# kvarq/kvarq

Measured on AMD Instinct MI355X. Metric: fastq_reads_per_sec_scanned, higher is better.
Workload: dtype u8

## Files before the change

### kvarq_amd/csrc/kernels_bp_pass.inc

```
#if BP_STRAIGHT
        {
            const uint32_t pass0 = 0;
#else
        for (uint32_t pass0 = 0; pass0 < nrec; pass0 += RP) {
#endif
            const uint32_t k = pass0 + gr;
            const bool have = k < nrec;
            uint32_t roff = 0; int rl = 0;
            constexpr bool late_probes = !BP_STRAIGHT && LG >= 0 && !DENSE;
            uint32_t c0, cp;
            if (have) {
                const uint32_t m = jn + 4u * k;
                const uint32_t rstart = m == 0 ? ST_PRE + (Ja & 15u) : (uint32_t)S.nl[m - 1] + 1u;
                const uint32_t n0 = S.nl[m], n1 = S.nl[m + 1], n2 = S.nl[m + 2], n3 = S.nl[m + 3];
                const uint32_t sread = n0 + 1u, plus = n1 + 1u, sscore = n2 + 1u;
        KVQ_MARK("trim" BP_SFX);
                if (gl == 0 && !late_probes) { if (dbg & 8u) { c0 = '@'; cp = '+'; } else { c0 = text[rstart]; cp = text[plus]; } }
                const int Q = (int)(n3 - sscore);
                const int per = (Q + (int)G - 1) >> lg;
                Seg sg; sg.beg = (int)mul_u24(gl, (uint32_t)per); if (sg.beg > Q) sg.beg = Q;
                int s1 = sg.beg + per; if (s1 > Q) s1 = Q;
                sg.len = 0; sg.pre = 0; sg.suf = 0; sg.best = 0; sg.bstart = sg.beg;
                {
                    auto round = [&](int c0_) -> Seg {
                        const int n = s1 - c0_ < 64 ? s1 - c0_ : 64;
                        const uint32_t bit = sscore + (uint32_t)c0_;
                        const uint32_t a = BP_LDS_GDP + ((bit >> 5) << 2), sh = bit & 31u;
                        const uint32_t d0 = lds_u32_at(a), d1 = lds_u32_at(a + 4u), d2 = lds_u32_at(a + 8u);
                        const uint64_t nmask = n < 64 ? (1ull << n) - 1ull : ~0ull;
                        const uint64_t mm = (((uint64_t)__builtin_amdgcn_alignbit(d2, d1, sh) << 32) | (uint64_t)__builtin_amdgcn_alignbit(d1, d0, sh)) & nmask;
                        Seg sub; sub.beg = c0_; sub.len = n;
                        int bs;
                        bp_runs64(mm, n, dbg, sub.pre, sub.suf, sub.best, bs);
                        sub.bstart = c0_ + bs;
                        return sub;
                    };
                    if (!__any(per > 64)) sg = round(sg.beg);
                    else {
                        for (int cc = sg.beg; cc < s1; cc += 64) {
                            const Seg sub = round(cc);
                            sg = (cc == sg.beg) ? sub : seg_merge(sg, sub);
                        }
                    }
                }
                if (G == 4u) {
#define KVQ_QUAD(v, ctl) __builtin_amdgcn_update_dpp(0, (v), (ctl), 0xf, 0xf, true)
                    {
                        Seg B;
                        B.len = KVQ_QUAD(sg.len, 0xB1); B.pre = KVQ_QUAD(sg.pre, 0xB1); B.suf = KVQ_QUAD(sg.suf, 0xB1);
                        B.best = KVQ_QUAD(sg.best, 0xB1); B.bstart = KVQ_QUAD(sg.bstart, 0xB1); B.beg = 0;
                        sg = seg_merge(sg, B);
                    }
                    {
                        Seg B;
                        B.len = KVQ_QUAD(sg.len, 0x4E); B.pre = KVQ_QUAD(sg.pre, 0x4E); B.suf = KVQ_QUAD(sg.suf, 0x4E);
                        B.best = KVQ_QUAD(sg.best, 0x4E); B.bstart = KVQ_QUAD(sg.bstart, 0x4E); B.beg = 0;
                        sg = seg_merge(sg, B);
                    }
                    rl = KVQ_QUAD(sg.best, 0x00);
                    roff = sread + (uint32_t)KVQ_QUAD(sg.bstart, 0x00);
#undef KVQ_QUAD
                } else {
                    for (uint32_t d = 1; d < G; d <<= 1) {
                        Seg B;
                        B.len = __shfl_xor(sg.len, (int)d, 64); B.pre = __shfl_xor(sg.pre, (int)d, 64); B.suf = __shfl_xor(sg.suf, (int)d, 64);
                        B.best = __shfl_xor(sg.best, (int)d, 64); B.bstart = __shfl_xor(sg.bstart, (int)d, 64); B.beg = 0;
                        if ((gl & d) == 0) sg = seg_merge(sg, B);
                    }
                    rl = __shfl(sg.best, lane & ~(int)(G - 1u), 64);
                    roff = sread + (uint32_t)__shfl(sg.bstart, lane & ~(int)(G - 1u), 64);
                }
                my_longest = my_longest > (uint32_t)(rl + 1) ? my_longest : (uint32_t)(rl + 1);
                if (gl == 0) {
                    if (rl < KVQ_RL_BINS && !recount) atomicAdd(&S.hist[rl >> 1], 1u << (16 * (rl & 1)));
                    S.rinfo[k] = roff | ((uint32_t)rl << 16);
                }
            }
        KVQ_MARK("trim end / filter" BP_SFX);
            BSTAMP(4);
            KVQ_SETPRIO(2);
            const uint32_t rpw = 64u >> lg, grw = (uint32_t)lane >> lg;
            const uint32_t wfirst = pass0 + wave * rpw;
            const uint32_t npass = wfirst < nrec ? (nrec - wfirst < rpw ? nrec - wfirst : rpw) : 0u;
            uint32_t *const q1 = S.q1 + wave * BP_QW; uint32_t *const q2 = S.q2 + wave * BP_Q2W;
            uint32_t sub = (dbg & 128u) ? npass : 0u, step = rpw;
#if BP_STRAIGHT
            if (sub < npass) {
#else
            while (sub < npass) {
#endif
                BTALLY(6, lane == 0);
                asm volatile("" : "+v"(rl), "+v"(roff));
                int minrl, me_; const __attribute__((address_space(1))) uint8_t *bmL;
                {
                    const BpArgsPtr A = bp_args(A_);
                    minrl = A->P.minreadlength; me_ = A->P.maxerrors;
                    bmL = (const __attribute__((address_space(1))) uint8_t *)A->X.bm1 + (1 << (2 * KK)) / 8;
                }
                const bool mine = have && rl >= minrl && !(dbg & 2u) && grw >= sub && grw - sub < step;
                uint32_t qn = 0;
                int e0 = 0, e1 = 0;
                if (mine) {
                    const int NPe = (rl - KK) / SS + 1;
                    const int per = (NPe + (int)G - 1) >> lg;
                    e0 = (int)mul_u24(gl, (uint32_t)per); if (e0 > NPe) e0 = NPe;
                    e1 = e0 + per; if (e1 > NPe) e1 = NPe;
                }
                auto fixed_block = [&](int pp, bool ok) -> bool {
                    const uint32_t code = cdp_code<KK>(roff + (uint32_t)(ok ? pp : 0));
                    const uint32_t bits = bmL[code >> 3];
                    return ok & (bool)((bits >> (code & 7u)) & 1u);
                };
                auto head_ok = [&](int jj) { return mine && jj <= me_ && (jj + 1) * KK <= rl; };
                auto tail_ok = [&](int jj) { const int pp = rl - (jj + 1) * KK; return mine && jj <= me_ && pp >= 0 && !((pp % KK) == 0 && pp <= me_ * KK); };
                const bool hhit = fixed_block((int)gl * KK, head_ok((int)gl));
                const bool thit = fixed_block(rl - ((int)gl + 1) * KK, tail_ok((int)gl));
                constexpr int NR = SS == 8 ? 6 : SS == 4 ? 12 : (LG == 3 || LG == 1) ? 24 : 18;
                bool first = true;
                if constexpr (!DENSE) {
                for (int ee = e0; __any(ee < e1); ee += NR, first = false) {
                    const bool act = ee < e1;
#include "kernels_bp_lookup.inc"
                    const int nv = act ? (e1 - ee < NR ? e1 - ee : NR) : 0;
                    hA &= (1u << nv) - 1u;
                    const bool hh = first && hhit, th = first && thit;
                    const uint32_t c = (uint32_t)__popc(hA) + (hh ? 1u : 0u) + (th ? 1u : 0u);
                    const uint32_t inc = kvq_wave_incl_scan(c);
                    const uint32_t tot = (uint32_t)__builtin_amdgcn_readlane((int)inc, 63);
                    if (tot) {
                        uint32_t idx = qn + inc - c;
                        while (hA) {
                            const int j = __ffs((int)hA) - 1; hA &= hA - 1u;
                            if (idx < BP_QW) q1[idx] = k | ((uint32_t)(SS * (ee + j)) << 9);
                            idx++;
                        }
                        if (hh) { if (idx < BP_QW) q1[idx] = k | ((gl * KK) << 9) | (1u << BP_Q1_KIND); idx++; }
                        if (th && idx < BP_QW) { const uint32_t pt = (uint32_t)(rl - ((int)gl + 1) * KK); q1[idx] = k | (pt << 9) | (1u << BP_Q1_KIND); }
                        qn += tot;
                    }
                }
                for (int t = (int)G; t <= me_; t += (int)G) {
                    const int jj = t + (int)gl;
#pragma unroll
                    for (int side = 0; side < 2; side++) {
                        const int pp = side ? rl - (jj + 1) * KK : jj * KK;
                        const bool hit = fixed_block(pp, side ? tail_ok(jj) : head_ok(jj));
                        const uint64_t mm = __ballot(hit);
                        if (mm) {
                            const uint32_t idx = qn + (uint32_t)__popcll(mm & kvq_lanemask_lt());
                            if (hit && idx < BP_QW) q1[idx] = k | ((uint32_t)pp << 9) | (1u << BP_Q1_KIND);
                            qn += (uint32_t)__popcll(mm);
                        }
                    }
                }
                }
        KVQ_MARK("filter end / P4a" BP_SFX);
                BSTAMP(5);
                KVQ_SETPRIO(3);

                if constexpr (!DENSE) {
                const bool over = qn > BP_QW;
                const uint32_t qn_ok = (over || (dbg & 1u)) ? 0u : qn;
#if BP_STRAIGHT
                if (over) bail = true;
                else {
#else
                if (over && step > 1u) { step >>= 1; continue; }
                if (over) {
                    if (mine && gl == 0) {
                        const BpArgsPtr A = bp_args(A_);
                        const KvqRedo Rd(A->redo);
                        const uint32_t boff = g0 - ST_PRE + roff;
                        bool put = false;
                        if (A->redo) {
                            if (rl >= KVQ_LONG_READ) {
                                const unsigned int i = atomicAdd(Rd.count + 1, 1u);
                                if (i < KVQ_LONG_CAP) { Rd.read_off[KVQ_REDO_CAP - 1u - i] = boff; Rd.read_len[KVQ_REDO_CAP - 1u - i] = rl; put = true; }
                            }
                            if (!put) {
                                const unsigned int i = atomicAdd(Rd.count, 1u);
                                if (i < A->redo_cap) { Rd.rec_start[i] = KVQ_REDO_TRIMMED; Rd.read_off[i] = boff; Rd.read_len[i] = rl; }
                                put = true;
                            }
                        }
                        if (!put) S.fallback = 1u;
                        else atomicOr(A->fail, 2u);
                    }
                }
#endif
#include "kernels_bp_p4.inc"
#if BP_STRAIGHT
                }
#endif
                } else {
                    uint32_t hA = 0, hpos = 0, tpos = 0; bool hh = false, th = false;
                    int ee = e0, xt = (int)G;
                    int ee_of_hA = e0;
                    bool done = false;
                    while (!done) {
                        bool full = false;
                        while (!full) {
                            if (!__any(hA != 0u || hh || th)) {
                                ee_of_hA = ee;
                                if (__any(ee < e1)) {
                                    const bool act = ee < e1;
                                    uint32_t hA_;
                                    {
#include "kernels_bp_lookup.inc"
                                        hA_ = hA;
                                    }
                                    const int nv = act ? (e1 - ee < NR ? e1 - ee : NR) : 0;
                                    hA = hA_ & ((1u << nv) - 1u);
                                    if (first) { hh = hhit; th = thit; hpos = gl * KK; tpos = (uint32_t)(rl - ((int)gl + 1) * KK); first = false; }
                                    ee += NR;
                                } else if (xt <= me_) {
                                    const int jj = xt + (int)gl;
                                    hpos = (uint32_t)(jj * KK); tpos = (uint32_t)(rl - (jj + 1) * KK);
                                    hh = fixed_block((int)hpos, head_ok(jj)); th = fixed_block((int)tpos, tail_ok(jj));
                                    xt += (int)G;
                                } else { done = true; break; }
                                continue;
                            }
                            const uint32_t c = (uint32_t)__popc(hA) + (hh ? 1u : 0u) + (th ? 1u : 0u);
                            const uint32_t inc = kvq_wave_incl_scan(c);
                            const uint32_t tot = (uint32_t)__builtin_amdgcn_readlane((int)inc, 63);
                            uint32_t idx = qn + inc - c;
                            while (hA && idx < BP_QW) {
                                const int j = __ffs((int)hA) - 1; hA &= hA - 1u;
                                q1[idx++] = k | ((uint32_t)(SS * (ee_of_hA + j)) << 9);
                            }
                            if (hh && idx < BP_QW) { q1[idx++] = k | (hpos << 9) | (1u << BP_Q1_KIND); hh = false; }
                            if (th && idx < BP_QW) { q1[idx++] = k | (tpos << 9) | (1u << BP_Q1_KIND); th = false; }
                            full = qn + tot >= BP_QW;
                            qn = qn + tot < BP_QW ? qn + tot : BP_QW;
                        }
                        {
                            const uint32_t qn_ok = (dbg & 1u) ? 0u : qn;
#include "kernels_bp_p4.inc"
                        }
                        qn = 0;
                    }
                }
                KVQ_SETPRIO(2);
                sub += step;
            }
            KVQ_SETPRIO(0);
            if (have && gl == 0) {
                const uint32_t m = jn + 4u * k;
                if constexpr (late_probes) {
                    if (!(dbg & 8u)) {
                        c0 = text[m == 0 ? ST_PRE + (Ja & 15u) : (uint32_t)S.nl[m - 1] + 1u];
                        cp = c0 == '@' ? (uint32_t)text[(uint32_t)S.nl[m + 1] + 1u] : (uint32_t)'+';
                    } else { c0 = '@'; cp = '+'; }
                }
                if (!bail && (c0 != '@' || cp != '+')) {
                    const BpArgsPtr A = bp_args(A_);
                    const uint32_t rstart = m == 0 ? ST_PRE + (Ja & 15u) : (uint32_t)S.nl[m - 1] + 1u, plus = (uint32_t)S.nl[m + 1] + 1u;
                    const int64_t tf = A->fpos_base + (int64_t)g0;
                    if (c0 != '@') atomicMin(A->P.err, ((unsigned long long)(tf + rstart - ST_PRE) << 16) | (0ull << 8) | c0);
                    else atomicMin(A->P.err, ((unsigned long long)(tf + plus - ST_PRE) << 16) | (1ull << 8) | cp);
                }
            }
        KVQ_MARK("P4 end" BP_SFX);
            BSTAMP(6);
        }
```

### kvarq_amd/csrc/kernels_seeded.hip

```cpp
#include "kvq_host.h"

#include <algorithm>
#include <string.h>

#ifdef KVQ_NO_PRIO
#define KVQ_SETPRIO(n) ((void)0)
#else
#define KVQ_SETPRIO(n) __builtin_amdgcn_s_setprio(n)
#endif
#define KVQ_K_MAX 8
#define ST_TILE 36640u
#define ST_TILE_MIN 30960u
#define ST_OV 4160u
#define ST_PRE 80u
#define ST_THREADS 512
#define ST_WAVES (ST_THREADS / 64)
#define ST_ROUNDS ((ST_TILE + ST_OV) / 16u / ST_THREADS + 1)
#define ST_NLCAP 2048
#define ST_RCAP 512
#define ST_QCAP 896
#define ST_Q2CAP 2048
#define ST_QW (ST_QCAP / ST_WAVES)
#define ST_Q2W (ST_Q2CAP / ST_WAVES)
#define ST_BLK 80u
#define ST_BUF (ST_PRE + ST_TILE + ST_OV)
#define ST_HIST_TILES 100u

#define TR_NONE 0xFFu
#define TR_FLAG_FALLBACK 0x2000000u
#define TR_FLAG_SKIPPED 0x4000000u
#define TR_FLAG_PARTIAL 0x8000000u
#define KVQ_SKIP_CAP 1024u

struct SeedEntry { uint64_t en, ctx; };
struct SeedTables {
    const uint32_t *bm1;
    const uint32_t *start;
    const SeedEntry *ent;
    const uint32_t *tab2;
    int32_t stride;
    int32_t pitch;
};

struct SeedIndex {
    int stride = 2;
    int k = 8;
    int pitch = 8;
    bool dense = false;
    DevBuf d_bm1, d_start, d_ent, d_tab2;
    SeedTables dev;
};

__host__ __device__ static inline uint32_t code2_of(uint8_t c) { return (c >> 1) & 3u; }

static uint32_t host_code(const uint8_t *p, int K)
{
    uint32_t c = 0;
    for (int i = 0; i < K; i++) c |= code2_of(p[i]) << (2 * i);
    return c;
}

int kvq_seed_k(const kvq_config &cfg)
{
    const int e = cfg.maxerrors;
    if (e < 0 || e > 6) return 0;
    if (cfg.Amin <= 13) return 0;
    int K = std::min(cfg.minoverlap, cfg.minreadlength) / (e + 1);
    if (K > KVQ_K_MAX) K = KVQ_K_MAX;
    if (const char *kv = getenv("KVQ_K")) { const int w = atoi(kv); if (w >= 5 && w < K) K = w; }
    return K >= 5 ? K : 0;
}

SeedIndex *kvq_seed_index_build(kvq_table *t)
{
    const kvq_config &cfg = t->cfg;
    t->seed_k = 0;
    const int e = cfg.maxerrors;
    const int K = kvq_seed_k(cfg);
    if (!K) return nullptr;
    auto pitch_of = [&](int stride) { return (K + stride - 1) / stride * stride; };
    auto span_of = [&](int stride) { return pitch_of(stride) * e + K + stride - 1; };
    int minlen = 1 << 30;
    for (int s = 0; s < t->nseq; s++) {
        const int len = t->h_off[s + 1] - t->h_off[s];
        bool ok = len >= span_of(2) && len <= 4095 && t->h_off[s] < (1 << 20) && s < (1 << 20);
        for (int i = 0; ok && i < len; i++) {
            const uint8_t c = t->h_tab[t->h_off[s] + i];
            ok = (c == 'A' || c == 'C' || c == 'G' || c == 'T');
        }
        if (ok) { t->seeded.push_back(s); t->is_seeded[s] = 1; minlen = std::min(minlen, len); }
    }
    if (t->seeded.empty()) return nullptr;
    t->seed_k = K;
    int stride = minlen >= span_of(8) ? 8 : minlen >= span_of(4) ? 4 : 2;
    if (const char *sv = getenv("KVQ_STRIDE")) { const int w = atoi(sv); if ((w == 2 || w == 4 || w == 8) && w <= stride) stride = w; }

    const int pitch = pitch_of(stride);
    struct Ent { uint32_t key; SeedEntry e; };
    std::vector<Ent> v;
    for (int s : t->seeded) {
        const uint8_t *q = &t->h_tab[t->h_off[s]];
        const int len = t->h_off[s + 1] - t->h_off[s];
        const uint64_t hi = ((uint64_t)(uint32_t)t->h_off[s] << 32) | ((uint64_t)(uint32_t)len << 52) | ((uint64_t)(uint32_t)s << 12);
        auto entry = [&](int pos, uint32_t all) -> Ent {
            uint64_t ctx = 0;
            for (int i = 0; i < 32; i++) { const int sp = pos - 16 + i; if (sp >= 0 && sp < len) ctx |= (uint64_t)code2_of(q[sp]) << (2 * i); }
            return Ent{ host_code(q + pos, K) + (all << (2 * K)), SeedEntry{ hi | (uint64_t)pos, ctx } };
        };
        for (int j = 0; j <= e; j++)
            for (int sft = 0; sft < stride; sft++) v.push_back(entry(j * pitch + sft, 0u));
        for (int p = 0; p + K <= len; p++) v.push_back(entry(p, 1u));
    }
    if (v.size() >= (1u << 22)) {
        t->seeded.clear(); std::fill(t->is_seeded.begin(), t->is_seeded.end(), 0); t->seed_k = 0;
        return nullptr;
    }
    SeedIndex *ix = new SeedIndex();
    ix->stride = stride; ix->k = K; ix->pitch = pitch;
    const uint32_t NC = 1u << (2 * K);
    std::vector<uint8_t> bm1(2 * NC / 8 < 64 ? 64 : 2 * NC / 8, 0);
    std::stable_sort(v.begin(), v.end(), [](const Ent &a, const Ent &b) { return a.key < b.key; });
    std::vector<uint32_t> start(2 * (size_t)NC + 2, 0); std::vector<SeedEntry> ent(v.size() + 1, SeedEntry{ 0, 0 });
    for (size_t i = 0; i < v.size(); i++) {
        bm1[v[i].key >> 3] |= (uint8_t)(1u << (v[i].key & 7));
        start[v[i].key + 1]++; ent[i] = v[i].e;
    }
    {
        size_t occ_anc = 0, occ_all = 0;
        for (uint32_t c = 0; c < NC; c++) { occ_anc += start[c + 1] != 0; occ_all += start[NC + c + 1] != 0; }
        const double expect = (double)occ_anc / NC * (150.0 / stride) + (double)occ_all / NC * 2 * (e + 1);
        ix->dense = expect > 5.0;
    }
    for (uint32_t c = 0; c < 2 * NC; c++) start[c + 1] += start[c];
    start[2 * (size_t)NC + 1] = start[2 * (size_t)NC];
    if (ix->d_start.ensure(start.size() * 4) != KVQ_OK || ix->d_ent.ensure(ent.size() * sizeof(SeedEntry)) != KVQ_OK ||
        hipMemcpy(ix->d_start.p, start.data(), start.size() * 4, hipMemcpyHostToDevice) != hipSuccess ||
        hipMemcpy(ix->d_ent.p, ent.data(), ent.size() * sizeof(SeedEntry), hipMemcpyHostToDevice) != hipSuccess ||
        ix->d_bm1.ensure(bm1.size()) != KVQ_OK || hipMemcpy(ix->d_bm1.p, bm1.data(), bm1.size(), hipMemcpyHostToDevice) != hipSuccess) {
        if (!kvq_error_code()) kvq_set_error(KVQ_ERR_DEVICE, "uploading the seed index failed");
        kvq_seed_index_destroy(ix);
        return nullptr;
    }
    ix->dev.bm1 = ix->d_bm1.as<uint32_t>();
    {
        const size_t nb = t->h_tab.size();
        std::vector<uint32_t> t2(nb / 16 + 3, 0);
        for (size_t i = 0; i < nb; i++) t2[i >> 4] |= code2_of(t->h_tab[i]) << (2 * (i & 15));
        if (ix->d_tab2.ensure(t2.size() * 4) != KVQ_OK || hipMemcpy(ix->d_tab2.p, t2.data(), t2.size() * 4, hipMemcpyHostToDevice) != hipSuccess) {
            if (!kvq_error_code()) kvq_set_error(KVQ_ERR_DEVICE, "uploading the seed index failed");
            kvq_seed_index_destroy(ix);
            return nullptr;
        }
        ix->dev.tab2 = ix->d_tab2.as<uint32_t>();
    }
    ix->dev.start = ix->d_start.as<uint32_t>(); ix->dev.ent = ix->d_ent.as<SeedEntry>();
    ix->dev.stride = stride; ix->dev.pitch = pitch;
    return ix;
}

void kvq_seed_index_destroy(SeedIndex *ix)
{
    if (!ix) return;
    DevBuf *b[] = { &ix->d_tab2, &ix->d_bm1, &ix->d_start, &ix->d_ent };
    for (DevBuf *x : b) x->release();
    delete ix;
}


__device__ __forceinline__ uint32_t lds_byte_at(uint32_t addr)
{
    return *reinterpret_cast<const __attribute__((address_space(3))) uint8_t *>((uintptr_t)addr);
}
__device__ __forceinline__ uint32_t rfl(uint32_t v) { return (uint32_t)__builtin_amdgcn_readfirstlane((int)v); }

typedef const __attribute__((address_space(1))) uint8_t *GlbBytes;
__device__ __forceinline__ uint32_t glb_u32(GlbBytes p)
{
    typedef uint32_t __attribute__((aligned(1))) u32_any;
    return *reinterpret_cast<const __attribute__((address_space(1))) u32_any *>(p);
}

__device__ __forceinline__ uint32_t good_flags(uint32_t x, uint32_t addk)
{
    return __builtin_amdgcn_bitop3_b32((x & 0x7F7F7F7Fu) + addk, 0x80808080u, x, 0x40);
}

__device__ __forceinline__ uint32_t mul_u24(uint32_t a, uint32_t b)
{
    uint32_t r;
    asm("v_mul_u32_u24 %0, %1, %2" : "=v"(r) : "v"(a), "v"(b));
    return r;
}

__device__ __forceinline__ void longest_run64(uint64_t m, int n, int &len, int &start)
{
    const uint64_t r1 = m & (m << 1), r2 = r1 & (r1 << 2), r3 = r2 & (r2 << 4), r4 = r3 & (r3 << 8), r5 = r4 & (r4 << 16);
    uint64_t E = n >= 64 ? ~0ull : ((1ull << n) - 1ull);
    int L = 0; uint64_t T;
    T = E & r5;        if (T) { E = T; L = 32; }
    T = E & (r4 << L); if (T) { E = T; L += 16; }
    T = E & (r3 << L); if (T) { E = T; L += 8; }
    T = E & (r2 << L); if (T) { E = T; L += 4; }
    T = E & (r1 << L); if (T) { E = T; L += 2; }
    T = E & (m << L);  if (T) { E = T; L += 1; }
    len = L;
    start = L ? (__ffsll((long long)E) - 1) - L + 1 : 0;
    if (m == ~0ull) { len = 64; start = 0; }
}

struct Seg { int len, pre, suf, best, bstart, beg; };

__device__ __forceinline__ Seg seg_merge(const Seg &A, const Seg &B)
{
    Seg R;
    R.beg = A.beg; R.len = A.len + B.len;
    R.pre = (A.pre == A.len) ? A.len + B.pre : A.pre;
    R.suf = (B.suf == B.len) ? B.len + A.suf : B.suf;
    R.best = A.best; R.bstart = A.bstart;
    const int cross = A.suf + B.pre;
    if (cross > R.best) { R.best = cross; R.bstart = A.beg + A.len - A.suf; }
    if (B.best > R.best) { R.best = B.best; R.bstart = B.bstart; }
    return R;
}

__device__ __forceinline__ int diff_bytes(uint32_t x, uint32_t y)
{
    const uint32_t v = x ^ y;
    return __popc(__builtin_amdgcn_bitop3_b32((v & 0x7F7F7F7Fu) + 0x7F7F7F7Fu, 0x80808080u, v, 0xC8));
}

__device__ __forceinline__ void emit_cold(const KvqParams *__restrict__ P, bool hit, int64_t fpos, int seq_nr,
                                          int seq_pos, int length, int rl, uint32_t key)
{
    const uint64_t m = __ballot(hit);
    if (m == 0) return;
    KvqHit *const arena = P->arena; const uint32_t cap = P->arena_cap; unsigned int *const arena_n = P->arena_n;
    const int leader = __ffsll((long long)m) - 1;
    uint32_t base = 0;
    if (kvq_lane() == leader) base = atomicAdd(arena_n, (unsigned int)__popcll(m));
    base = __shfl(base, leader, 64);
    if (hit) {
        const uint32_t idx = base + (uint32_t)__popcll(m & kvq_lanemask_lt());
        if (idx < cap) {
            KvqHit h;
            h.fpos = fpos; h.seq_nr = seq_nr; h.seq_pos = seq_pos; h.length = length;
            h.readlength = rl; h.key = key; h.blob_off = 0;
            arena[idx] = h;
        }
    }
}

#define ST_NO_BLOCK 0x7FFFFF00u
__host__ __device__ static inline bool kvq_tile_report_bad(uint32_t rep, bool first_tile, uint32_t seen, uint32_t total)
{
    const uint32_t n_owned = rep & 0xFFFFu, jn = (rep >> 16) & 0xFFu;
    if (rep & TR_FLAG_FALLBACK) return true;
    if ((rep & TR_FLAG_SKIPPED) && !(rep & TR_FLAG_PARTIAL)) return false;
    const uint32_t want = first_tile ? 0u : 4u - (seen & 3u);
    const bool expect = want <= n_owned && (first_tile || want + 2u <= total - seen);
    return expect ? jn != want : jn != TR_NONE;
}

extern "C" __global__ void __launch_bounds__(256)
kvq_validate_tiles(uint32_t nchunks, const uint32_t *__restrict__ tile_first, const uint32_t *__restrict__ tile_report,
                   unsigned int *__restrict__ spec_fail, KvqSkippedTile *__restrict__ skip_list,
                   const uint32_t *__restrict__ chunk_off, uint32_t tile_bytes)
{
    KVQ_BESIDE_SCAN();
    const uint32_t c = blockIdx.x * blockDim.x + threadIdx.x;
    if (c >= nchunks) return;
    uint32_t total = 0;
    for (uint32_t g = tile_first[c]; g < tile_first[c + 1]; g++) total += tile_report[g] & 0xFFFFu;
    uint32_t seen = 0;
    bool bad = false;
    for (uint32_t g = tile_first[c]; g < tile_first[c + 1]; g++) {
        const uint32_t rep = tile_report[g];
        if (kvq_tile_report_bad(rep, g == tile_first[c], seen, total)) bad = true;
        if ((rep & TR_FLAG_SKIPPED) && skip_list) {
            const unsigned int k = atomicAdd(spec_fail, 0x100u) >> 8;
            if (k < KVQ_SKIP_CAP) {
                const uint32_t a = chunk_off[c], e = chunk_off[c + 1], tn = g - tile_first[c];
                const uint32_t g0 = (a & ~15u) + tn * tile_bytes;
                KvqSkippedTile T;
                T.a = a; T.b = e; T.own_begin = tn == 0 ? a : g0; T.own_end = (uint64_t)g0 + tile_bytes < e ? g0 + tile_bytes : e;
                T.seen = seen; T.first = tn == 0 ? 1u : 0u;
                const uint32_t z = tile_report[tile_first[nchunks] + g];
                if (z) { T.a = T.own_begin = z - 1u; T.seen = 0; T.first = 1u; }
                skip_list[k] = T;
            } else bad = true;
        }
        seen += rep & 0xFFFFu;
    }
    if (bad) atomicOr(spec_fail, 1u);
}


extern "C" __global__ void __launch_bounds__(256)
kvq_expand_tiles(uint32_t nchunks, const uint32_t *__restrict__ chunk_off, const uint32_t *__restrict__ tile_first, uint4 *__restrict__ tile_tab, unsigned int *__restrict__ redo_count,
                 unsigned int *__restrict__ surv_count)
{
    KVQ_BESIDE_SCAN();
    const uint32_t c = blockIdx.x * blockDim.x + threadIdx.x;
    if (c == 0 && redo_count) { redo_count[0] = 0; redo_count[1] = 0; }
    if (c == 0 && surv_count) surv_count[0] = 0;
    if (c >= nchunks) return;
    const uint32_t a = chunk_off[c], b = chunk_off[c + 1], g0 = tile_first[c];
    for (uint32_t g = g0; g < tile_first[c + 1]; g++) tile_tab[g] = make_uint4(a, b, g - g0, c);
}

uint32_t kvq_choose_tile(uint32_t maxline, uint32_t rec_bytes)
{
    if (const char *e = getenv("KVQ_TILE")) { const int v = atoi(e); if (v >= 4000 && v <= (int)(ST_TILE + ST_OV - 1040u)) return (uint32_t)v / ST_BLK * ST_BLK; }
    if (maxline == 0) return ST_TILE;
    uint32_t ov = (4u * (maxline + 2u) + 160u + ST_BLK - 1u) / ST_BLK * ST_BLK;
    ov = std::max<uint32_t>(1040u, std::min<uint32_t>(ov, ST_OV));
    uint32_t tile = ST_TILE + ST_OV - ov;
    if (rec_bytes >= 40u) {
        const uint32_t n_full = tile / rec_bytes + 1u;
        uint32_t p = 1; while (2u * p <= n_full) p *= 2u;
        if (p >= 16u && p <= (uint32_t)ST_THREADS && n_full > p) {
            const uint32_t cut = (p - 1u) * rec_bytes / ST_BLK * ST_BLK;
            if (cut >= ST_TILE_MIN && (uint64_t)cut * 100u >= (uint64_t)tile * 78u) tile = cut;
        }
    }
    return tile;
}
uint32_t kvq_min_tile()
{
    if (getenv("KVQ_TILE")) return std::min<uint32_t>(ST_TILE_MIN, kvq_choose_tile(1u << 20, 0));
    return ST_TILE_MIN;
}

void kvq_probe_text(const uint8_t *text, size_t n, uint32_t &maxline, uint32_t &rec_bytes)
{
    uint32_t best = 0; size_t start = 0, lines = 0;
    for (size_t i = 0; i < n; i++)
        if (text[i] == '\n') { best = std::max<uint32_t>(best, (uint32_t)(i + 1 - start)); start = i + 1; lines++; }
    maxline = std::max<uint32_t>(best, (uint32_t)(n - start));
    rec_bytes = lines >= 16 ? (uint32_t)(start * 4 / lines) : 0u;
}
extern "C" uint32_t kvq_tile_for_text(const uint8_t *text, size_t n, uint32_t *rec_bytes_out)
{
    uint32_t maxline, rec_bytes;
    kvq_probe_text(text, n, maxline, rec_bytes);
    if (rec_bytes_out) *rec_bytes_out = rec_bytes;
    return kvq_choose_tile(maxline, rec_bytes);
}
```

Baseline: 10.01 billion.

## Replace lane-group segment merge with packed prefix-scan and max-key reduction

Replaces the per-lane Seg merge reduction, which shuffles five fields per step, with a packed 32-bit encoding. A suffix scan over the following segments' prefix-run words computes how far each lane's trailing run extends. Each lane then proposes a packed (length, start) key, and a single-word max reduction over DPP row or xor shuffles selects the winner. This cuts cross-lane traffic and ALU work in the trim stage, at the cost of a subtler encoding whose tie-breaking and 16-bit field limits must match the old semantics.

```diff
diff --git a/kvarq_amd/csrc/kernels_bp_pass.inc b/kvarq_amd/csrc/kernels_bp_pass.inc
--- a/kvarq_amd/csrc/kernels_bp_pass.inc
+++ b/kvarq_amd/csrc/kernels_bp_pass.inc
@@ -43,33 +43,35 @@
                         }
                     }
                 }
-                if (G == 4u) {
-#define KVQ_QUAD(v, ctl) __builtin_amdgcn_update_dpp(0, (v), (ctl), 0xf, 0xf, true)
-                    {
-                        Seg B;
-                        B.len = KVQ_QUAD(sg.len, 0xB1); B.pre = KVQ_QUAD(sg.pre, 0xB1); B.suf = KVQ_QUAD(sg.suf, 0xB1);
-                        B.best = KVQ_QUAD(sg.best, 0xB1); B.bstart = KVQ_QUAD(sg.bstart, 0xB1); B.beg = 0;
-                        sg = seg_merge(sg, B);
-                    }
-                    {
-                        Seg B;
-                        B.len = KVQ_QUAD(sg.len, 0x4E); B.pre = KVQ_QUAD(sg.pre, 0x4E); B.suf = KVQ_QUAD(sg.suf, 0x4E);
-                        B.best = KVQ_QUAD(sg.best, 0x4E); B.bstart = KVQ_QUAD(sg.bstart, 0x4E); B.beg = 0;
-                        sg = seg_merge(sg, B);
-                    }
-                    rl = KVQ_QUAD(sg.best, 0x00);
-                    roff = sread + (uint32_t)KVQ_QUAD(sg.bstart, 0x00);
-#undef KVQ_QUAD
+                uint32_t key;
+                if constexpr (LG >= 0) {
+                    static_assert(LG <= 4, "a lane group is at most a DPP row");
+#define KVQ_ROW(v, ctl) (uint32_t)__builtin_amdgcn_update_dpp(0, (int)(v), (ctl), 0xf, 0xf, true)
+                    uint32_t x = KVQ_ROW(kvq_tm_word(sg.pre, sg.len), 0x101);
+                    if (s1 == Q) x = KVQ_TM_STOP;
+                    if constexpr (LG >= 2) { x = kvq_tm_combine(x, KVQ_ROW(x, 0x101)); x = kvq_tm_combine(x, KVQ_ROW(x, 0x102)); }
+                    if constexpr (LG >= 3) x = kvq_tm_combine(x, KVQ_ROW(x, 0x104));
+                    if constexpr (LG >= 4) x = kvq_tm_combine(x, KVQ_ROW(x, 0x108));
+                    key = kvq_tm_proposal(sg, s1, kvq_tm_ext(x));
+                    uint32_t o;
+                    if constexpr (LG >= 1) { o = KVQ_ROW(key, 0xB1); key = key > o ? key : o; }
+                    if constexpr (LG >= 2) { o = KVQ_ROW(key, 0x4E); key = key > o ? key : o; }
+                    if constexpr (LG >= 3) { o = KVQ_ROW(key, 0x141); key = key > o ? key : o; }
+                    if constexpr (LG >= 4) { o = KVQ_ROW(key, 0x140); key = key > o ? key : o; }
+#undef KVQ_ROW
                 } else {
-                    for (uint32_t d = 1; d < G; d <<= 1) {
-                        Seg B;
-                        B.len = __shfl_xor(sg.len, (int)d, 64); B.pre = __shfl_xor(sg.pre, (int)d, 64); B.suf = __shfl_xor(sg.suf, (int)d, 64);
-                        B.best = __shfl_xor(sg.best, (int)d, 64); B.bstart = __shfl_xor(sg.bstart, (int)d, 64); B.beg = 0;
-                        if ((gl & d) == 0) sg = seg_merge(sg, B);
-                    }
-                    rl = __shfl(sg.best, lane & ~(int)(G - 1u), 64);
-                    roff = sread + (uint32_t)__shfl(sg.bstart, lane & ~(int)(G - 1u), 64);
-                }
+                    uint32_t Gw = G; asm volatile("" : "+s"(Gw));
+                    uint32_t x = (uint32_t)__shfl_down((int)kvq_tm_word(sg.pre, sg.len), 1, 64);
+                    if (s1 == Q) x = KVQ_TM_STOP;
+                    for (uint32_t d = 1; d + 1u < Gw; d <<= 1) x = kvq_tm_combine(x, (uint32_t)__shfl_down((int)x, (int)d, 64));
+                    key = kvq_tm_proposal(sg, s1, kvq_tm_ext(x));
+                    for (uint32_t d = 1; d < Gw; d <<= 1) {
+                        const uint32_t o = (uint32_t)__shfl_xor((int)key, (int)d, 64);
+                        key = key > o ? key : o;
+                    }
+                }
+                rl = kvq_tm_length(key);
+                roff = sread + kvq_tm_start(key);
                 my_longest = my_longest > (uint32_t)(rl + 1) ? my_longest : (uint32_t)(rl + 1);
                 if (gl == 0) {
                     if (rl < KVQ_RL_BINS && !recount) atomicAdd(&S.hist[rl >> 1], 1u << (16 * (rl & 1)));
diff --git a/kvarq_amd/csrc/kernels_seeded.hip b/kvarq_amd/csrc/kernels_seeded.hip
--- a/kvarq_amd/csrc/kernels_seeded.hip
+++ b/kvarq_amd/csrc/kernels_seeded.hip
@@ -208,20 +208,7 @@
     if (m == ~0ull) { len = 64; start = 0; }
 }
 
-struct Seg { int len, pre, suf, best, bstart, beg; };
-
-__device__ __forceinline__ Seg seg_merge(const Seg &A, const Seg &B)
-{
-    Seg R;
-    R.beg = A.beg; R.len = A.len + B.len;
-    R.pre = (A.pre == A.len) ? A.len + B.pre : A.pre;
-    R.suf = (B.suf == B.len) ? B.len + A.suf : B.suf;
-    R.best = A.best; R.bstart = A.bstart;
-    const int cross = A.suf + B.pre;
-    if (cross > R.best) { R.best = cross; R.bstart = A.beg + A.len - A.suf; }
-    if (B.best > R.best) { R.best = B.best; R.bstart = B.bstart; }
-    return R;
-}
+#include "kvq_trim_merge.h"
 
 __device__ __forceinline__ int diff_bytes(uint32_t x, uint32_t y)
 {
diff --git a/kvarq_amd/csrc/kvq_trim_merge.h b/kvarq_amd/csrc/kvq_trim_merge.h
--- /dev/null
+++ b/kvarq_amd/csrc/kvq_trim_merge.h
@@ -0,0 +1,46 @@
+#pragma once
+#include <stdint.h>
+
+#if defined(__HIPCC__)
+#define KVQ_TM_HD __host__ __device__ __forceinline__
+#else
+#define KVQ_TM_HD inline
+#endif
+
+struct Seg { int len, pre, suf, best, bstart, beg; };
+
+KVQ_TM_HD Seg seg_merge(const Seg &A, const Seg &B)
+{
+    Seg R;
+    R.beg = A.beg; R.len = A.len + B.len;
+    R.pre = (A.pre == A.len) ? A.len + B.pre : A.pre;
+    R.suf = (B.suf == B.len) ? B.len + A.suf : B.suf;
+    R.best = A.best; R.bstart = A.bstart;
+    const int cross = A.suf + B.pre;
+    if (cross > R.best) { R.best = cross; R.bstart = A.beg + A.len - A.suf; }
+    if (B.best > R.best) { R.best = B.best; R.bstart = B.bstart; }
+    return R;
+}
+
+#define KVQ_TM_STOP 0xC0000000u
+
+KVQ_TM_HD uint32_t kvq_tm_word(int pre, int len) { return ((uint32_t)(pre - len) << 16) + (uint32_t)pre; }
+KVQ_TM_HD uint32_t kvq_tm_combine(uint32_t a, uint32_t b)
+{
+    uint32_t t = a + b;
+#if defined(__HIP_DEVICE_COMPILE__)
+    asm("" : "+v"(t));
+#endif
+    return (int32_t)a >= 0 ? t : a;
+}
+KVQ_TM_HD int kvq_tm_ext(uint32_t w) { return (int)(w & 0xFFFFu); }
+
+KVQ_TM_HD uint32_t kvq_tm_key(int length, int start) { return ((uint32_t)length << 16) | (0xFFFFu - (uint32_t)start); }
+KVQ_TM_HD int kvq_tm_length(uint32_t key) { return (int)(key >> 16); }
+KVQ_TM_HD uint32_t kvq_tm_start(uint32_t key) { return ~key & 0xFFFFu; }
+
+KVQ_TM_HD uint32_t kvq_tm_proposal(const Seg &s, int end, int ext)
+{
+    const uint32_t inside = kvq_tm_key(s.best, s.bstart), across = kvq_tm_key(s.suf + ext, end - s.suf);
+    return inside > across ? inside : across;
+}
```

Measured after the change: 10.05 billion, median of 6. Within noise of the previous version (+0.4%).
